# pk17r/online_3d_reconstruction

Measured on AMD Instinct MI355X. Metric: frames_per_sec, higher is better.
Workload: dtype f32; 1 GPU; synthetic 1280x720 dense stereo, jump_pixels 1, 200 frames/GPU, voxel_size 0.05, min_points_per_voxel 1, SOR off, frames resident in HBM (BASELINE.json configs[1]); frames_per_gpu=200, rows=720, cols=1280, jump_pixels=1, parallelism=frame-sharded x1

## Files before the change

### online_3d_reconstruction_amd/csrc/kernels/radix_sort.inc

```

__device__ __forceinline__ int64_t hist_at(bool tm, int dgt, int tile, int n_tiles)
{
    return tm ? (int64_t)tile * kMaxRadix + dgt : (int64_t)dgt * n_tiles + tile;
}

__global__ __launch_bounds__(kSortThreads) void k_radix_hist(const uint32_t* __restrict__ keys0,
                                                             const uint32_t* __restrict__ keys1, int64_t cap,
                                                             const VoxelGeom* __restrict__ geom, int pass,
                                                             int n_tiles, uint32_t* __restrict__ hist,
                                                             uint32_t* __restrict__ hist_part, int tm)
{
    constexpr int kSub = 4;
    __shared__ uint32_t h[kSub * kSortWaves * kMaxRadix];
    const int f = blockIdx.y, tile = blockIdx.x;
    const VoxelGeom g = geom[f];
    if (g.overflow || pass >= (int)g.passes) return;
    const uint32_t n = g.n;
    if ((int64_t)tile * kSortTile >= (int64_t)n) return;
    const int bins = geom_bins(g), shift = pass * (int)g.bpp;
    const uint32_t dmask = (uint32_t)bins - 1u;
    for (int i = threadIdx.x; i < kSub * kSortWaves * kMaxRadix; i += kSortThreads) h[i] = 0;
    __syncthreads();
    const uint32_t* src = (((pass + g.buf0) & 1) ? keys1 : keys0) + (int64_t)f * cap;
    const int64_t base = (int64_t)tile * kSortTile;
// ... 83 lines not shown
            dst[i] = key;
            atomicAdd(&hw[key & dmask], 1u);
        }
    }
    __syncthreads();
    uint32_t* hd = hist + (int64_t)f * kMaxRadix * n_tiles;
    for (int dgt = threadIdx.x; dgt < bins; dgt += kSortThreads) {
        uint32_t t = 0;
#pragma unroll
        for (int ww = 0; ww < kSub * kSortWaves; ++ww) t += h[ww * kMaxRadix + dgt];
        hd[hist_at(tm != 0, dgt, tile, n_tiles)] = t;
    }
}

constexpr int kCntStride = 17;
constexpr int kCntWords = kMaxRadix * kCntStride;
constexpr int kRankWords = kScatWaves * kCntWords;
struct ScatterLds {
    __attribute__((aligned(16))) uint32_t smem[kRankWords > 2 * kScatTile ? kRankWords : 2 * kScatTile];
    uint32_t wave_tot[kScatWaves * kMaxRadix];
    uint32_t local_base[kMaxRadix];
    uint32_t delta[kMaxRadix];
    uint32_t scan_lds[kScatWaves + 1];
};
struct ScatterJob {
    const uint32_t *kin, *vin;
    uint32_t *kout, *vout;
    const uint32_t* hist;
    const uint32_t* hist_part;
    int64_t begin, end;
    uint32_t dmask;
    int shift, bins, pass, n_tiles;
    bool tm;
};

__device__ __forceinline__ void emit_part_range(const uint32_t* __restrict__ tile_off, int n_emit_tiles, int tile, int part,
                                                int64_t n, int64_t& begin, int64_t& end)
{
    if (tile_off) {
        constexpr int kPer = kEmitGroup / kScatParts;
        const int e0 = (tile * kScatParts + part) * kPer;
        begin = tile_off[e0];
        end = e0 + kPer < n_emit_tiles ? (int64_t)tile_off[e0 + kPer] : n;
    } else {
        begin = (int64_t)tile * kSortTile + (int64_t)part * kScatTile;
        end = begin + kScatTile < n ? begin + kScatTile : n;
    }
}
typedef uint32_t u32x4_a4_t __attribute__((ext_vector_type(4), aligned(4)));

__device__ __forceinline__ void scatter_load(const ScatterJob& J, int tile, int part, uint32_t (&key)[kSortRounds],
                                             uint32_t (&val)[kSortRounds], uint32_t& gstart)
{
    const int lane = threadIdx.x & 63, w = threadIdx.x >> 6;
    const int64_t lbase = J.begin + (int64_t)w * kSortWaveItems + (int64_t)lane * kSortRounds;
    gstart = 0;
    if ((int)threadIdx.x < J.bins) {
        gstart = J.hist[hist_at(J.tm, threadIdx.x, tile, J.n_tiles)];
        if (part != 0) gstart += J.hist_part[hist_at(J.tm, threadIdx.x, tile, J.n_tiles)];
    }
    if (lbase + kSortRounds <= J.end) {
#pragma unroll
        for (int q = 0; q < kSortRounds / 4; ++q) {
            const u32x4_a4_t k4 = *reinterpret_cast<const u32x4_a4_t*>(J.kin + lbase + 4 * q);
            key[4 * q] = k4.x; key[4 * q + 1] = k4.y; key[4 * q + 2] = k4.z; key[4 * q + 3] = k4.w;
        }
        if (J.pass != 0) {
#pragma unroll
            for (int q = 0; q < kSortRounds / 4; ++q) {
                const u32x4_a4_t v4 = *reinterpret_cast<const u32x4_a4_t*>(J.vin + lbase + 4 * q);
                val[4 * q] = v4.x; val[4 * q + 1] = v4.y; val[4 * q + 2] = v4.z; val[4 * q + 3] = v4.w;
            }
        }
    } else {
#pragma unroll
        for (int r = 0; r < kSortRounds; ++r) {
            const int64_t i = lbase + r;
            const bool ok = i < J.end;
            key[r] = ok ? J.kin[i] : 0xffffffffu;
            val[r] = (J.pass != 0 && ok) ? J.vin[i] : 0u;
        }
    }
    if (J.pass == 0) {
#pragma unroll
        for (int r = 0; r < kSortRounds; ++r) val[r] = (uint32_t)(lbase + r);
    }
}

__device__ __forceinline__ void scatter_tile(const ScatterJob& J, ScatterLds& L, const uint32_t (&key)[kSortRounds],
                                             const uint32_t (&val)[kSortRounds], uint32_t gstart)
{
    uint32_t* smem = L.smem;
    uint32_t* stage = L.smem;
    const int lane = threadIdx.x & 63, w = threadIdx.x >> 6;
    const uint32_t cnt = (uint32_t)(J.end - J.begin);
    const int64_t lbase = J.begin + (int64_t)w * kSortWaveItems + (int64_t)lane * kSortRounds;
    const int shift = J.shift, bins = J.bins;
    const uint32_t dmask = J.dmask;
    for (int i = threadIdx.x; i < kRankWords; i += kScatThreads) smem[i] = 0;
    __syncthreads();

    uint32_t* cw = smem + w * kCntWords;
    const int quad = lane >> 2, sub = lane & 3;
    const uint32_t fsh = 7u * (uint32_t)sub;
    uint32_t own[kSortRounds];
#pragma unroll
    for (int r = 0; r < kSortRounds; ++r) {
        own[r] = 0;
        if (lbase + r < J.end) {
            const uint32_t dgt = (key[r] >> shift) & dmask;
            const uint32_t old = atomicAdd(&cw[dgt * kCntStride + quad], 1u << fsh);
            own[r] = (old >> fsh) & 127u;
        }
    }
    __builtin_amdgcn_wave_barrier();
#pragma unroll
    for (int h = 0; h < kMaxRadix / 64; ++h) {
        const int row = lane + 64 * h;
        if (row < bins) {
            uint32_t run = 0;
#pragma unroll
            for (int j = 0; j < 16; ++j) {
                const uint32_t v = cw[row * kCntStride + j];
                const uint32_t t = v + (v << 7);
                const uint32_t t2 = t + (t << 14);
                cw[row * kCntStride + j] = (run << 21) | (t2 & 0x1fffffu);
                run += (t2 >> 21) & 127u;
            }
            L.wave_tot[w * kMaxRadix + row] = run;
        }
    }
    __syncthreads();

    uint32_t tot = 0;
    const int dg = threadIdx.x;
    if (dg < bins) {
#pragma unroll
        for (int ww = 0; ww < kScatWaves; ++ww) {
            const uint32_t t = L.wave_tot[ww * kMaxRadix + dg];
            L.wave_tot[ww * kMaxRadix + dg] = tot;
            tot += t;
        }
    }
    uint32_t tile_total;
    const uint32_t lb = block_excl_scan_u32<kScatWaves>(tot, L.scan_lds, tile_total);
    if (dg < bins) {
        L.local_base[dg] = lb;
        L.delta[dg] = gstart - lb;
    }
    __syncthreads();

    uint32_t pos[kSortRounds];
    const uint32_t qsh = sub ? 7u * (uint32_t)(sub - 1) : 0u, qmk = sub ? 127u : 0u;
#pragma unroll
    for (int r = 0; r < kSortRounds; ++r) {
        if (lbase + r < J.end) {
            const uint32_t dgt = (key[r] >> shift) & dmask;
            const uint32_t v = cw[dgt * kCntStride + quad];
            pos[r] = L.local_base[dgt] + L.wave_tot[w * kMaxRadix + dgt] + (v >> 21) + ((v >> qsh) & qmk) + own[r];
        }
    }
    __syncthreads();
    uint32_t* stage_v = L.smem + kScatTile;
#pragma unroll
    for (int r = 0; r < kSortRounds; ++r) {
        if (lbase + r < J.end) {
            stage[pos[r]] = key[r];
            stage_v[pos[r]] = val[r];
        }
    }
    __syncthreads();
#pragma unroll
    for (int r = 0; r < kSortRounds; ++r) {
        const uint32_t p = r * kScatThreads + threadIdx.x;
        if (p < cnt) {
            const uint32_t k = stage[p];
            const uint32_t d = p + L.delta[(k >> shift) & dmask];
            J.kout[d] = k;
            J.vout[d] = stage_v[p];
        }
    }
}

__global__ __launch_bounds__(kScatThreads) void k_radix_scatter_lane(uint32_t* __restrict__ keys0, uint32_t* __restrict__ vals0,
                                                                     uint32_t* __restrict__ keys1, uint32_t* __restrict__ vals1,
                                                                     int64_t cap, const VoxelGeom* __restrict__ geom, int pass,
                                                                     int n_tiles, const uint32_t* __restrict__ hist_scanned,
                                                                     const uint32_t* __restrict__ hist_part, int tm,
                                                                     const uint32_t* __restrict__ emit_tile_off,
                                                                     int n_emit_tiles)
{
    __shared__ ScatterLds L;
    const int f = blockIdx.y;
    const VoxelGeom g = geom[f];
    if (g.overflow || pass >= (int)g.passes) return;
    const uint32_t* tile_off = emit_tile_off ? emit_tile_off + (int64_t)f * n_emit_tiles : nullptr;
    const int n_items = tile_off ? (n_emit_tiles + kEmitGroup / kScatParts - 1) / (kEmitGroup / kScatParts)
                                 : (int)(((int64_t)g.n + kScatTile - 1) / kScatTile);
    const int item = xcd_chunk_item(blockIdx.x, n_items);
    if (item < 0) return;
    const int tile = item / kScatParts, part = item % kScatParts;
    ScatterJob J;
    emit_part_range(tile_off, n_emit_tiles, tile, part, (int64_t)g.n, J.begin, J.end);
    if (J.begin >= J.end) return;
    const int par = (pass + (int)g.buf0) & 1;
    J.kin = (par ? keys1 : keys0) + (int64_t)f * cap;
    J.vin = (par ? vals1 : vals0) + (int64_t)f * cap;
    J.kout = (par ? keys0 : keys1) + (int64_t)f * cap;
    J.vout = (par ? vals0 : vals1) + (int64_t)f * cap;
    J.hist = hist_scanned + (int64_t)f * kMaxRadix * n_tiles;
    J.hist_part = hist_part + (int64_t)f * kMaxRadix * n_tiles;
    J.bins = geom_bins(g);
    J.dmask = (uint32_t)J.bins - 1u;
    J.shift = pass * (int)g.bpp;
    J.pass = pass;
    J.n_tiles = n_tiles;
    J.tm = tm != 0;
    uint32_t key0[kSortRounds], val0[kSortRounds], g0;
    scatter_load(J, tile, part, key0, val0, g0);
    scatter_tile(J, L, key0, val0, g0);
}
```

### online_3d_reconstruction_amd/csrc/kernels/voxel_runs.inc

```


constexpr int kHeadWaves = 4;
__global__ __launch_bounds__(kHeadWaves * kWave) void k_run_heads(const uint32_t* __restrict__ keys0, const uint32_t* __restrict__ keys1,
                                                                  int64_t cap, const VoxelGeom* __restrict__ geom, int n_tiles,
                                                                  uint32_t* __restrict__ seg_cnt, int buf_sel,
                                                                  uint8_t* __restrict__ head_bits)
{
    static_assert(kSegTile == 16 * kWave, "16 records per lane");
    const int f = blockIdx.y, lane = threadIdx.x & 63;
    const int tile = blockIdx.x * kHeadWaves + (threadIdx.x >> 6);
    const VoxelGeom g = geom[f];
    if (g.overflow || tile >= n_tiles) return;
    const int64_t n = g.n;
    const uint32_t* k = (buf_sel < 0 ? sorted_buf(g, keys0, keys1) : (buf_sel ? keys1 : keys0)) + (int64_t)f * cap;
    uint32_t c = 0;
    const int64_t i0 = (int64_t)tile * kSegTile + lane * 16;
    if ((int64_t)tile * kSegTile < n) {
        uint32_t kk[16];
        if (((((int64_t)f * cap) & 3) == 0) && i0 + 15 < n) {
#pragma unroll
            for (int q = 0; q < 4; ++q) {
                const uint4 v = *reinterpret_cast<const uint4*>(k + i0 + 4 * q);
                kk[4 * q] = v.x; kk[4 * q + 1] = v.y; kk[4 * q + 2] = v.z; kk[4 * q + 3] = v.w;
            }
        } else {
#pragma unroll
            for (int q = 0; q < 16; ++q) kk[q] = (i0 + q < n) ? k[i0 + q] : 0u;
        }
        uint32_t prev = (uint32_t)wave_shr1_i32((int32_t)kk[15]);
        if (lane == 0) prev = (i0 > 0 && i0 < n) ? k[i0 - 1] : 0u;
        uint32_t bits = 0;
#pragma unroll
        for (int q = 0; q < 16; ++q) {
            const int64_t i = i0 + q;
            if (i < n && (i == 0 || kk[q] != (q ? kk[q - 1] : prev))) bits |= 1u << ((q >> 2) * 8 + (q & 3));
        }
        reinterpret_cast<uint32_t*>(head_bits + ((int64_t)f * n_tiles + tile) * 256)[lane] = bits;
        c = (uint32_t)__popc(bits);
    }
    c = wave_sum_u32(c);
    if (lane == 0) seg_cnt[(int64_t)f * n_tiles + tile] = c;
}

constexpr int kStartWaves = 4;
__global__ __launch_bounds__(kStartWaves * kWave) void k_run_starts(
    const uint32_t* __restrict__ keys0, const uint32_t* __restrict__ keys1, int64_t cap, const VoxelGeom* __restrict__ geom,
    int n_tiles, const uint32_t* __restrict__ seg_off, const uint32_t* __restrict__ n_vox, uint32_t* __restrict__ seg_start,
    int buf_sel, uint32_t* __restrict__ head_keys_out, const VoxelGeom* __restrict__ mode, const o3dr_point* __restrict__ in_pts,
    float z_offset, const uint8_t* __restrict__ head_bits)
{
    static_assert(kSegTile == 16 * kWave, "16 records per lane");
    const int f = blockIdx.y, lane = threadIdx.x & 63;
    const int tile = blockIdx.x * kStartWaves + (threadIdx.x >> 6);
    const VoxelGeom g = geom[f];
    if (g.overflow) return;
    if (mode && mode[f].grouped == 0u) return;
    const uint32_t n = g.n;
    const int64_t base = (int64_t)tile * kSegTile;
// ... 64 lines not shown
    const int f = blockIdx.y, tile = blockIdx.x;
    if (geom[f].overflow || geom[f].grouped != 0u) return;
    const uint32_t nv = n_vox[f];
    const int64_t base = (int64_t)tile * kSegTile;
    if (base >= nv) return;
    const uint32_t* ss = seg_start + (int64_t)f * (cap + 1);
    uint32_t* ki = keep_idx + (int64_t)f * cap;
    uint32_t off = seg_off[(int64_t)f * n_tiles + tile];
    for (int j = 0; j < kSegTile / 256; ++j) {
        const int64_t o = base + j * 256 + threadIdx.x;
        const bool keep = (o < nv) && (ss[o + 1] - ss[o] >= min_points);
        uint32_t total;
        const uint32_t pos = block_excl_scan_u32<4>(keep ? 1u : 0u, scan_lds, total);
        if (keep) ki[off + pos] = (uint32_t)o;
        off += total;
    }
}

__global__ __launch_bounds__(256) void k_frame_offsets(const VoxelGeom* __restrict__ geom, const uint32_t* __restrict__ n_vox,
                                                       const uint32_t* __restrict__ n_keep,
                                                       const uint32_t* __restrict__ n_grp, int frames, int passthrough,
                                                       uint32_t* __restrict__ n_out, uint64_t* __restrict__ out_off,
                                                       CloudCounters* __restrict__ cc, SortStats* __restrict__ stats,
                                                       const VoxelGeom* __restrict__ sort_geom)
{
    __shared__ uint32_t scan_lds[5];
    __shared__ unsigned long long acc[6];
    if (threadIdx.x < 6) acc[threadIdx.x] = 0;
    __syncthreads();
    const uint64_t base = cc->count;
    uint64_t carry = 0;
    for (int f0 = 0; f0 < frames; f0 += 256) {
        const int f = f0 + threadIdx.x;
        uint32_t m = 0;
        if (f < frames) {
            const VoxelGeom g = geom[f];
            if (passthrough) {
                m = g.n;
            } else if (g.overflow) {
                m = g.n;
                atomicOr(&acc[3], (unsigned long long)O3DR_STATUS_VOXEL_OVERFLOW);
            } else {
                m = (n_grp && sort_geom[f].grouped) ? n_grp[f] : (n_keep ? n_keep[f] : n_vox[f]);
                atomicAdd(&acc[0], (unsigned long long)sort_geom[f].n * g.passes);
                atomicAdd(&acc[5], (unsigned long long)sort_geom[f].n);
                atomicAdd(&acc[1], (unsigned long long)g.n);
                atomicAdd(&acc[2], (unsigned long long)m);
            }
        }
        uint32_t total;
        const uint32_t excl = block_excl_scan_u32<4>(m, scan_lds, total);
        if (f < frames) {
            n_out[f] = m;
            out_off[f] = base + carry + excl;
        }
        carry += total;
    }
    __syncthreads();
    if (threadIdx.x == 0) {
        cc->count = base + carry;
        cc->status |= (uint32_t)acc[3];
        if (stats) {
            stats->sort_record_passes += acc[0];
            stats->voxel_points_in += acc[1];
            stats->voxel_points_out += acc[2];
            stats->sort_records += acc[5];
        }
    }
}

__global__ void k_test_corrupt_payload(uint32_t* __restrict__ vals0, uint32_t* __restrict__ vals1, const VoxelGeom* __restrict__ geom)
{
    const VoxelGeom g = geom[0];
    if (g.overflow || g.n == 0u) return;
    uint32_t* v = ((g.passes + g.buf0) & 1u) ? vals1 : vals0;
    v[g.n / 2u] = 0xfffffff0u;
}

__device__ __forceinline__ void centroid_block(int64_t bx, int f, const VoxelGeom& g, uint32_t n_o,
                                               const o3dr_point* __restrict__ in, int64_t in_fstride,
                                               const uint32_t* __restrict__ vals0, const uint32_t* __restrict__ vals1,
                                               int64_t cap, const uint32_t* __restrict__ seg_start,
                                               const uint32_t* __restrict__ keep_idx, const uint64_t* __restrict__ out_off,
                                               float z_offset, int passthrough, o3dr_point* __restrict__ out_base,
                                               float* __restrict__ out_mm, int nbx, CloudCounters* __restrict__ cc,
                                               const CloudHeads& ch)
{
    const int64_t o = bx * kPtThreads + threadIdx.x;
    const bool active = o < (int64_t)n_o;
// ... 418 lines not shown
```

### online_3d_reconstruction_amd/csrc/o3dr_api.hip

```cpp
#include <dlfcn.h>
#include <stdio.h>
#include <stdlib.h>
#include <string.h>

#include <algorithm>
#include <cfloat>
#include <chrono>
#include <cmath>
#include <condition_variable>
#include <mutex>
#include <string>
#include <vector>

#include <rccl/rccl.h>

#include "../../include/o3dr_testing.h"
#include "o3dr_device.h"
#include "o3dr_image_stack.h"
#include "o3dr_profile.h"

using namespace o3dr;

static thread_local std::string g_err;
static int fail(int code, const char* what)
// ... 193 lines not shown
        sort_tiles > c->ws_sort_tiles || seg_tiles > c->ws_seg_tiles || mm_floats > c->ws_mm_floats) {
        const size_t MM = mm_floats > c->ws_mm_floats ? mm_floats : c->ws_mm_floats;
        const size_t E = elems > c->ws_elems ? elems : c->ws_elems;
        const int F = frames > c->ws_frames ? frames : c->ws_frames;
        const size_t TE = emit_tiles > c->ws_emit_tiles ? emit_tiles : c->ws_emit_tiles;
        const size_t TS = sort_tiles > c->ws_sort_tiles ? sort_tiles : c->ws_sort_tiles;
        const size_t TG = seg_tiles > c->ws_seg_tiles ? seg_tiles : c->ws_seg_tiles;
        Workspace& w = c->ws;
        const size_t boxes = E / 64 + 8 * (size_t)F + 64;
        CHK(carve(c, c->ws_block, [&](Carve& k) {
            k.take(w.keys[0], E);
            k.take(w.keys[1], E);
            k.take(w.vals[0], E);
            k.take(w.vals[1], E);
            k.take(w.seg_start, E);
            k.take(w.keep_idx, E);
            k.take(w.run_start, E);
            k.take(w.grp_cnt, (E > (size_t)kGroupMinSlots ? E : (size_t)kGroupMinSlots) / kGroupCells + 2);
            k.take(w.tile_cnt, TE);
            k.take(w.hist, TS * kMaxRadix);
            k.take(w.hist_part, TS * kMaxRadix);
            k.take(w.seg_cnt, TG);
            k.take(w.head_bits, TG * 256);
            k.take(w.scan_partial, (TS * kMaxRadix + TG + TE + E) / 4096 + 8 * (size_t)F + 16);
            k.take(w.mm, MM);
            k.take(w.n_valid, (size_t)F);
            k.take(w.n_kp, (size_t)F);
            k.take(w.n_vox, (size_t)F);
            k.take(w.n_out, (size_t)F);
            k.take(w.out_off, (size_t)F);
            k.take(w.geom, (size_t)F);
            k.take(w.geom_runs, (size_t)F);
            k.take(w.n_runs, (size_t)F);
            k.take(w.n_grp_out, (size_t)F);
            k.take(w.out_mm, boxes * 6);
            k.take(w.out_mm_partial, (size_t)kBoxFoldBlocks * 6);
            k.take(w.wave_gc, boxes * 6);
            w.bytes = k.off;
        }));
        c->ws_elems = E;
        c->ws_frames = F;
        c->ws_emit_tiles = TE;
        c->ws_sort_tiles = TS;
        c->ws_seg_tiles = TG;
        c->ws_mm_floats = MM;
    }
// ... 1279 lines not shown
            launch_reproject(&c->prof, c->stream, a, nb, c->ws.pts, c->ws.tile_cnt, c->ws.n_kp, c->ws.n_valid, c->ws.mm,
                             c->ws.scan_partial);
        VoxelArgs v;
        v.keys_ready = fused ? 1 : 0;
        v.emit_tiles = emit_tiles;
        v.cloud_box = c->cloud_box_valid ? c->cloud_box : nullptr;
        heads_for_append(c, v);
        v.in = c->ws.pts;
        v.in_fstride = cap;
        v.n_dev = c->ws.n_valid;
        v.frames = nb;
        v.cap = cap;
        v.leaf[0] = leaf[0];
        v.leaf[1] = leaf[1];
        v.leaf[2] = leaf[2];
        v.min_points = mp;
        v.z_offset = zo;
        v.out_base = c->cloud_big;
        v.cc = c->cc_big;
        v.passthrough = c->params.dont_downsample ? 1 : 0;
        v.mm_used = a.n_tiles + 1;
        v.stats = c->stats_dev;
        v.use_runs = 0;
        if (with_sor) {
            v.mm_used = launch_sor(&c->prof, c->stream, c->ws, c->ws.pts, cap, c->ws.n_valid, nb, cap, a.n_tiles + 1, 1.0, c->ws.sor_pts,
                                   cap, c->ws.sor_n);
            v.in = c->ws.sor_pts;
            v.n_dev = c->ws.sor_n;
        }
        launch_voxel_grid(&c->prof, c->stream, c->ws, v);
        HIPCHK(hipGetLastError());
        c->cloud_ub += (int64_t)nb * cap;
        c->cloud_n_exact = false;
        if (streaming) HIPCHK(hipEventRecord(c->ev_done[slot], c->stream));
    }
    if (streaming) HIPCHK(hipStreamSynchronize(c->stream));
    return O3DR_OK;
}

extern "C" int o3dr_accumulate_frames(o3dr_ctx* c, const uint8_t* disp, int64_t disp_frame_stride, int64_t disp_pitch,
                                      const uint8_t* bgr, int64_t bgr_frame_stride, int64_t bgr_pitch, int32_t rows,
                                      int32_t cols, const float* poses, int32_t n_frames, int32_t mem)
{
    return accumulate_impl(c, disp, disp_frame_stride, disp_pitch, bgr, bgr_frame_stride, bgr_pitch, rows, cols, poses, n_frames,
                           nullptr, nullptr, mem);
}
// ... 3902 lines not shown
    if (total_ms) *total_ms = c->prof.total_ms[kernel_id];
    if (launches) *launches = c->prof.launches[kernel_id];
    return O3DR_OK;
}
extern "C" int o3dr_profile_reset(o3dr_ctx* c)
{
    CTX_ENTER(c);
    HIPCHK(hipMemsetAsync(c->stats_dev, 0, sizeof(SortStats), c->stream));
    HIPCHK(hipStreamSynchronize(c->stream));
    c->prof.reset();
    return O3DR_OK;
}
extern "C" int o3dr_profile_stats(o3dr_ctx* c, int64_t out[8])
{
    CTX_ENTER(c);
    if (!out) return fail(O3DR_ERR_INVALID_ARG, "out is NULL");
    HIPCHK(hipMemcpyAsync(c->stats_host, c->stats_dev, sizeof(SortStats), hipMemcpyDeviceToHost, c->stream));
    HIPCHK(hipStreamSynchronize(c->stream));
    out[0] = (int64_t)c->stats_host->sort_record_passes;
    out[1] = (int64_t)c->stats_host->voxel_points_in;
    out[2] = (int64_t)c->stats_host->voxel_points_out;
    out[3] = 0;
    out[4] = (int64_t)c->stats_host->sort_records;
    out[5] = out[6] = out[7] = 0;
    return O3DR_OK;
}
extern "C" int o3dr_device_info(o3dr_ctx* c, char* name, int32_t name_len, int32_t* cu_count, int64_t* hbm_bytes)
{
    CTX_ENTER(c);
    hipDeviceProp_t p;
    HIPCHK(hipGetDeviceProperties(&p, c->device));
    if (name && name_len > 0) snprintf(name, (size_t)name_len, "%s (%s)", p.name, p.gcnArchName);
    if (cu_count) *cu_count = p.multiProcessorCount;
    if (hbm_bytes) *hbm_bytes = (int64_t)p.totalGlobalMem;
    return O3DR_OK;
}
```

### online_3d_reconstruction_amd/csrc/o3dr_device.h

```cpp
#pragma once
#include <hip/hip_runtime.h>
#include <stdint.h>

#include "../../include/o3dr.h"

namespace o3dr {

constexpr int kWave = 64;
constexpr int kEmitThreads = 256;
constexpr int kEmitPerLane = 4;
constexpr int kEmitTile = kEmitThreads * kEmitPerLane;
constexpr int kSortWaves = 8;
constexpr int kSortThreads = kSortWaves * kWave;
constexpr int kSortRounds = 16;
constexpr int kSortWaveItems = kSortRounds * kWave;
constexpr int kSortTile = kSortWaves * kSortWaveItems;
constexpr int kScatParts = 2;
constexpr int kScatWaves = kSortWaves / kScatParts;
constexpr int kScatThreads = kScatWaves * kWave;
constexpr int kScatTile = kScatWaves * kSortWaveItems;
constexpr int kEmitGroup = kSortTile / kEmitTile;
static_assert(kEmitGroup * kEmitTile == kSortTile && kEmitGroup % kScatParts == 0, "a scatter part is a whole number of emit tiles");
constexpr int kMaxRadixBits = 7;
constexpr int kMaxRadix = 1 << kMaxRadixBits;
constexpr int kMaxPasses = 5;
static_assert(kMaxRadix <= 2 * kSortThreads, "k_radix_scatter handles two digits per thread");
constexpr int kSlabClasses = 4;
constexpr int kXcds = 8;
constexpr int kPtThreads = 256;
constexpr int kSegTile = 1024;
constexpr int kMinmaxBlocks = 1024;
constexpr int kPartWords = 8;
constexpr int kSmallMax = 8192;
constexpr int kGroupBits = 5;
constexpr int kGroupCells = 1 << kGroupBits;
static_assert(kGroupCells <= kWave, "one lane per voxel of a group");
constexpr int kGroupWaves = 4;
constexpr int kGroupMinRunNum = 5, kGroupMinRunDen = 4;
constexpr int64_t kGroupMinCloud = 1 << 20;
constexpr int64_t kGroupMinSlots = 1 << 20;

struct VoxelGeom {
    float inv[3];
    int32_t min_b[3];
    int32_t div_b[3];
    uint32_t mul1, mul2;
    uint32_t overflow;
    uint32_t n;
    uint32_t passes;
// ... 34 lines not shown
    double min_disp;
    int32_t min_disp_u8;
    int64_t out_fstride;
    int64_t mm_stride;
    const QLutEntry* lut;
    int32_t disp_f64;
    float slab_inv[3];
    int32_t slab_shift;
};

struct Workspace {
    int32_t frames = 0;
    int64_t cap = 0;
    int32_t n_emit_tiles = 0, n_sort_tiles = 0, n_seg_tiles = 0;
    o3dr_point* pts = nullptr;
    uint32_t* keys[2] = {nullptr, nullptr};
    uint32_t* vals[2] = {nullptr, nullptr};
    uint32_t* seg_start = nullptr;
    uint32_t* tile_cnt = nullptr;
    uint32_t* hist = nullptr;
    uint32_t* hist_part = nullptr;
    uint32_t* seg_cnt = nullptr;
    uint8_t* head_bits = nullptr;
    uint32_t* scan_partial = nullptr;
    SorGeom* sor_geom = nullptr;
    float4* sor_xyz = nullptr;
    float* sor_dist = nullptr;
    uint32_t* sor_cell_first = nullptr;
    float2* sor_cell_z = nullptr;
    uint32_t sor_max_cells = 0;
    double* sor_partial = nullptr;
    o3dr_point* sor_pts = nullptr;
    uint32_t* sor_n = nullptr;
    uint32_t* sor_left = nullptr;
    uint32_t* sor_left_cnt = nullptr;
    int64_t sor_cap = 0;
    uint32_t* keep_idx = nullptr;
    uint32_t* run_start = nullptr;
    uint32_t* grp_cnt = nullptr;
    int64_t grp_slots = 0;
    uint32_t* n_runs = nullptr;
    uint32_t* n_grp_out = nullptr;
    VoxelGeom* geom_runs = nullptr;
    float* out_mm = nullptr;
    float* out_mm_partial = nullptr;
    int32_t* wave_gc = nullptr;
    float* mm = nullptr;
    int64_t mm_stride = 0;
    uint32_t* n_valid = nullptr;
    uint32_t* n_kp = nullptr;
    uint32_t* n_vox = nullptr;
    uint32_t* n_out = nullptr;
    uint64_t* out_off = nullptr;
    VoxelGeom* geom = nullptr;
    size_t bytes = 0;
};

struct SortStats {
    uint64_t sort_record_passes;
    uint64_t voxel_points_in;
    uint64_t voxel_points_out;
    uint64_t reserved;
    uint64_t sort_records;
    uint64_t pad[3];
};

struct CloudHeads {
    uint32_t* flags;
    float inv[3];
    float z_offset;
    int32_t* wave_gc;
};

struct CloudCounters {
    uint64_t count;
    uint32_t status;
    uint32_t pad;
};

struct IncGroup {
    int32_t bx, iy, iz;
    uint32_t mask;
};
struct IncCell {
    float s[7];
    uint32_t n;
};
// ... 461 lines not shown
```

### online_3d_reconstruction_amd/csrc/o3dr_kernels.hip

```cpp
#include <string.h>

#include "o3dr_device.h"
#include "o3dr_profile.h"

namespace o3dr {

#include "kernels/util.inc"
#include "kernels/reproject.inc"
#include "kernels/bookkeeping.inc"
#include "kernels/prepass.inc"
#include "kernels/voxel_index.inc"
#include "kernels/radix_sort.inc"
#include "kernels/voxel_runs.inc"
#include "kernels/incremental.inc"
#include "kernels/multigpu.inc"
#include "kernels/sor.inc"
#include "kernels/small.inc"
#include "kernels/nn.inc"
#include "kernels/mls.inc"
#include "kernels/cell_order.inc"
#include "kernels/plane.inc"
#include "kernels/mesh.inc"
#include "kernels/raster.inc"
#include "kernels/match.inc"
// ... 231 lines not shown
            }
            {
                ProfScope ps(pf, O3DR_K_OTHER, s);
                launch_scan(s, ws.seg_cnt, n_seg_tiles, n_seg_tiles, F, ws.n_runs, nullptr, ws.scan_partial);
            }
            {
                ProfScope ps(pf, O3DR_K_SEGMENT, s);
                k_run_geom<<<cdiv64(F, 64), 64, 0, s>>>(ws.geom, ws.n_runs, F, ws.geom_runs, v.use_runs > 1 ? 1 : 0, grp_slots);
                k_run_starts<<<dim3(cdiv64(n_seg_tiles, kStartWaves), F), kStartWaves * kWave, 0, s>>>(
                    ws.keys[0], ws.keys[1], cap, ws.geom, n_seg_tiles, ws.seg_cnt, ws.n_runs, ws.run_start, 0, ws.keys[1],
                    ws.geom_runs, v.in, v.z_offset, hb);
            }
            {
                ProfScope ps(pf, O3DR_K_KEYGEN, s);
                k_voxel_keys_hist0<<<grid, kSortThreads, 0, s>>>(v.in, v.in_fstride, ws.geom, v.z_offset, cap, ws.keys[0],
                                                                 n_sort_tiles, ws.hist, ws.hist_part, ws.geom_runs, tm);
            }
        } else if (!v.keys_ready) {
            ProfScope ps(pf, O3DR_K_KEYGEN, s);
            k_voxel_keys_hist0<<<grid, kSortThreads, 0, s>>>(v.in, v.in_fstride, ws.geom, v.z_offset, cap, ws.keys[0],
                                                             n_sort_tiles, ws.hist, ws.hist_part, nullptr, tm);
        }
        const int64_t hist_row = (int64_t)kMaxRadix * n_sort_tiles;

        for (int pass = 0; pass < kMaxPasses; ++pass) {
            const bool emit_tiles = pass == 0 && v.emit_tiles > 0;
            if (!(pass == 0 && ((!use_runs && !v.keys_ready) || emit_tiles))) {
                ProfScope ps(pf, O3DR_K_SORT_HIST, s);
                k_radix_hist<<<grid, kSortThreads, 0, s>>>(ws.keys[0], ws.keys[1], cap, sort_geom, pass, n_sort_tiles,
                                                          ws.hist, ws.hist_part, tm);
            }
            {
                ProfScope ps(pf, O3DR_K_OTHER, s);
                if (tm)
                    k_scan_hist_tm<<<F, 1024, tm_lds, s>>>(ws.hist, sort_geom, pass, n_sort_tiles, emit_tiles ? 1 : 0);
                else
                    launch_scan(s, ws.hist, hist_row, hist_row, F, nullptr, nullptr, ws.scan_partial, sort_geom, pass,
                                n_sort_tiles);
            }
            {
                ProfScope ps(pf, O3DR_K_SORT_SCATTER, s);
                k_radix_scatter_lane<<<dim3(xcd_grid((int64_t)n_sort_tiles * kScatParts), F), kScatThreads, 0, s>>>(
                    ws.keys[0], ws.vals[0], ws.keys[1], ws.vals[1], cap, sort_geom, pass, n_sort_tiles, ws.hist, ws.hist_part, tm,
                    emit_tiles ? ws.tile_cnt : nullptr, v.emit_tiles);
            }
        }
        const dim3 sgrid(n_seg_tiles, F);
        {
            ProfScope ps(pf, O3DR_K_SEGMENT, s);
            k_run_heads<<<dim3(cdiv64(n_seg_tiles, kHeadWaves), F), kHeadWaves * kWave, 0, s>>>(ws.keys[0], ws.keys[1], cap, sort_geom, n_seg_tiles,
                                                                                       ws.seg_cnt, -1, ws.head_bits);
        }
        {
            ProfScope ps(pf, O3DR_K_OTHER, s);
            launch_scan(s, ws.seg_cnt, n_seg_tiles, n_seg_tiles, F, ws.n_vox, nullptr, ws.scan_partial);
        }
        {
            ProfScope ps(pf, O3DR_K_SEGMENT, s);
            k_run_starts<<<dim3(cdiv64(n_seg_tiles, kStartWaves), F), kStartWaves * kWave, 0, s>>>(ws.keys[0], ws.keys[1], cap, sort_geom, n_seg_tiles, ws.seg_cnt, ws.n_vox,
                                              ws.seg_start, -1, nullptr, nullptr, nullptr, 0.f, ws.head_bits);
        }
        if (v.min_points > 1) {
            {
                ProfScope ps(pf, O3DR_K_SEGMENT, s);
                k_keep_count<<<sgrid, 256, 0, s>>>(ws.seg_start, cap, sort_geom, ws.n_vox, v.min_points, n_seg_tiles, ws.seg_cnt);
            }
            {
                ProfScope ps(pf, O3DR_K_OTHER, s);
                launch_scan(s, ws.seg_cnt, n_seg_tiles, n_seg_tiles, F, ws.n_out, nullptr, ws.scan_partial);
            }
            {
                ProfScope ps(pf, O3DR_K_SEGMENT, s);
                k_keep_write<<<sgrid, 256, 0, s>>>(ws.seg_start, cap, sort_geom, ws.n_vox, v.min_points, n_seg_tiles, ws.seg_cnt,
                                                  ws.keep_idx);
// ... 5 lines not shown
        k_test_corrupt_payload<<<1, 1, 0, s>>>(ws.vals[0], ws.vals[1], sort_geom);
    if (cap > 0 && use_runs) {
        {
            ProfScope ps(pf, O3DR_K_OTHER, s);
            (void)hipMemsetAsync(ws.grp_cnt, 0, sizeof(uint32_t) * (size_t)(max_groups + 1), s);
        }
        {
            ProfScope ps(pf, O3DR_K_CENTROID_RUNS, s);
            int64_t nwg = cdiv64(max_groups < cap ? max_groups : cap, kGroupWaves);
            if (nwg > 16384) nwg = 16384;
            if (nwg < 1) nwg = 1;
            k_centroid_groups<<<(int)nwg, kGroupWaves * kWave, 0, s>>>(
                v.in, ws.keys[0], ws.keys[1], ws.vals[0], ws.vals[1], ws.seg_start, ws.run_start, ws.geom_runs, ws.geom, ws.n_vox,
                v.z_offset, v.min_points, reinterpret_cast<uint4*>(ws.pts), grp_slots, ws.grp_cnt, v.cc);
        }
        {
            ProfScope ps(pf, O3DR_K_OTHER, s);
            launch_scan(s, ws.grp_cnt, max_groups + 1, max_groups + 1, 1, ws.n_grp_out, nullptr, ws.scan_partial);
        }
    }
    {
        ProfScope ps(pf, O3DR_K_OTHER, s);
        k_frame_offsets<<<1, 256, 0, s>>>(ws.geom, ws.n_vox, n_keep, use_runs ? ws.n_grp_out : nullptr, F, v.passthrough,
                                          ws.n_out, ws.out_off, v.cc, v.stats, sort_geom);
    }
    const int nbx = cdiv64(cap, kPtThreads);
    if (cap > 0 && use_runs) {
        ProfScope ps(pf, O3DR_K_CENTROID_RUNS, s);
        int64_t nwg = cdiv64(cap, 256);
        if (nwg > 8192) nwg = 8192;
        k_group_compact<<<(int)nwg, 256, 0, s>>>(v.in, ws.geom_runs, ws.geom, ws.n_vox, ws.grp_cnt,
                                                reinterpret_cast<const uint4*>(ws.pts), ws.out_off, v.z_offset, v.out_base);
    }
    if (cap > 0) {
        ProfScope ps(pf, O3DR_K_CENTROID, s);
        float* out_mm = v.cloud_box ? ws.out_mm : nullptr;
        CloudHeads heads = v.cloud_heads;
        heads.wave_gc = ws.wave_gc;
        const uint32_t* keep = (v.min_points > 1 && !v.passthrough) ? ws.keep_idx : nullptr;
        if (use_runs)
            k_centroid<true><<<dim3(nbx < 4096 ? nbx : 4096, F), kPtThreads, 0, s>>>(
                v.in, v.in_fstride, ws.vals[0], ws.vals[1], cap, ws.seg_start, keep, ws.geom_runs, ws.n_out, ws.out_off,
                v.z_offset, v.passthrough, v.out_base, out_mm, nbx, v.cc, CloudHeads{nullptr, {0.f, 0.f, 0.f}, 0.f, nullptr});
        else
            k_centroid<false><<<dim3(xcd_grid(nbx), F), kPtThreads, 0, s>>>(
                v.in, v.in_fstride, ws.vals[0], ws.vals[1], cap, ws.seg_start, keep, ws.geom, ws.n_out, ws.out_off,
                v.z_offset, v.passthrough, v.out_base, out_mm, nbx, v.cc, heads);
// ... 41 lines not shown
        ProfScope ps(pf, O3DR_K_SEGMENT, s);
        k_run_geom<<<1, 64, 0, s>>>(ws.geom, ws.n_runs, 1, ws.geom_runs, 1, INT64_MAX);
        k_run_starts<<<dim3(cdiv64(n_seg_tiles, kStartWaves), 1), kStartWaves * kWave, 0, s>>>(
            ws.keys[0], ws.keys[1], cap, ws.geom, n_seg_tiles, ws.seg_cnt, ws.n_runs, ws.run_start, 0, ws.keys[1], ws.geom_runs, in,
            z_offset, ws.head_bits);
    }
    const dim3 grid(n_sort_tiles, 1);
    const int64_t hist_row = (int64_t)kMaxRadix * n_sort_tiles;
    for (int pass = 0; pass < kMaxPasses; ++pass) {
        {
            ProfScope ps(pf, O3DR_K_SORT_HIST, s);
            k_radix_hist<<<grid, kSortThreads, 0, s>>>(ws.keys[0], ws.keys[1], cap, sort_geom, pass, n_sort_tiles, ws.hist, ws.hist_part, tm);
        }
        {
            ProfScope ps(pf, O3DR_K_OTHER, s);
            if (tm)
                k_scan_hist_tm<<<1, 1024, tm_lds, s>>>(ws.hist, sort_geom, pass, n_sort_tiles, 0);
            else
                launch_scan(s, ws.hist, hist_row, hist_row, 1, nullptr, nullptr, ws.scan_partial, sort_geom, pass, n_sort_tiles);
        }
        {
            ProfScope ps(pf, O3DR_K_SORT_SCATTER, s);
            k_radix_scatter_lane<<<dim3(xcd_grid((int64_t)n_sort_tiles * kScatParts), 1), kScatThreads, 0, s>>>(
                ws.keys[0], ws.vals[0], ws.keys[1], ws.vals[1], cap, sort_geom, pass, n_sort_tiles, ws.hist, ws.hist_part, tm, nullptr, 0);
        }
    }
    {
        ProfScope ps(pf, O3DR_K_SEGMENT, s);
        k_run_heads<<<dim3(cdiv64(n_seg_tiles, kHeadWaves), 1), kHeadWaves * kWave, 0, s>>>(ws.keys[0], ws.keys[1], cap, sort_geom,
                                                                                             n_seg_tiles, ws.seg_cnt, -1, ws.head_bits);
    }
    {
        ProfScope ps(pf, O3DR_K_OTHER, s);
        launch_scan(s, ws.seg_cnt, n_seg_tiles, n_seg_tiles, 1, ws.n_vox, nullptr, ws.scan_partial);
    }
    {
        ProfScope ps(pf, O3DR_K_SEGMENT, s);
        k_run_starts<<<dim3(cdiv64(n_seg_tiles, kStartWaves), 1), kStartWaves * kWave, 0, s>>>(
            ws.keys[0], ws.keys[1], cap, sort_geom, n_seg_tiles, ws.seg_cnt, ws.n_vox, ws.seg_start, -1, nullptr, nullptr, nullptr, 0.f,
            ws.head_bits);
    }
    if (test_corrupt) k_test_corrupt_payload<<<1, 1, 0, s>>>(ws.vals[0], ws.vals[1], sort_geom);
}

void launch_inc_fold(Profiler* pf, hipStream_t s, Workspace& ws, const o3dr_point* in, float z_offset, const IncFoldArgs& a,
                     uint32_t* partial)
{
    {
        ProfScope ps(pf, O3DR_K_CENTROID_RUNS, s);
        int64_t nwg = cdiv64(a.nt, kGroupWaves);
        if (nwg > 16384) nwg = 16384;
        if (nwg < 1) nwg = 1;
        k_inc_fold<<<(int)nwg, kGroupWaves * kWave, 0, s>>>(in, ws.keys[0], ws.keys[1], ws.vals[0], ws.vals[1], ws.seg_start, ws.run_start,
// ... 343 lines not shown
}
void launch_partition(Profiler* pf, hipStream_t s, Workspace& ws, const VoxelArgs& v, int n_parts, o3dr_point* out,
                      uint64_t* counts_dev, uint32_t* overflow_dev, const void* hdrs_dev, int n_hdrs)
{
    launch_partition_count(pf, s, ws, v, n_parts, counts_dev, overflow_dev, hdrs_dev, n_hdrs);
    launch_partition_move(pf, s, ws, v, n_parts, out, nullptr);
}

static void launch_radix_passes(Workspace& ws, hipStream_t s, int64_t cap, int passes, int frames = 1)
{
    const int F = frames;
    const int n_sort_tiles = cdiv64(cap, kSortTile);
    const int64_t hist_row = (int64_t)kMaxRadix * n_sort_tiles;
    const size_t tm_lds = hist_tm_lds(n_sort_tiles);
    const int tm = hist_tm(n_sort_tiles);
    for (int pass = 0; pass < passes && pass < kMaxPasses; ++pass) {
        k_radix_hist<<<dim3(n_sort_tiles, F), kSortThreads, 0, s>>>(ws.keys[0], ws.keys[1], cap, ws.geom, pass, n_sort_tiles, ws.hist,
                                                                    ws.hist_part, tm);
        if (tm)
            k_scan_hist_tm<<<F, 1024, tm_lds, s>>>(ws.hist, ws.geom, pass, n_sort_tiles, 0);
        else
            launch_scan(s, ws.hist, hist_row, hist_row, F, nullptr, nullptr, ws.scan_partial, ws.geom, pass, n_sort_tiles);
        k_radix_scatter_lane<<<dim3(xcd_grid((int64_t)n_sort_tiles * kScatParts), F), kScatThreads, 0, s>>>(
            ws.keys[0], ws.vals[0], ws.keys[1], ws.vals[1], cap, ws.geom, pass, n_sort_tiles, ws.hist, ws.hist_part, tm, nullptr, 0);
    }
}

void launch_search_grid(Workspace& ws, hipStream_t s, const o3dr_point* in, int64_t in_fstride, const uint32_t* n_dev, int frames,
                        int64_t cap, int mm_used, double cell_points, uint32_t active_above)
{
    const int F = frames;
    const int64_t cell_stride = (int64_t)ws.sor_max_cells + 1;
    uint32_t max_cells = (uint32_t)(cap / 2 > 1024 ? cap / 2 : 1024);
    if (max_cells > ws.sor_max_cells) max_cells = ws.sor_max_cells;
    int cell_bits = 1;
    while ((1u << cell_bits) < max_cells) ++cell_bits;
    const int sort_passes = (cell_bits + kMaxRadixBits - 1) / kMaxRadixBits;
    k_sor_plan<<<F, 256, 0, s>>>(ws.mm, ws.mm_stride, mm_used, n_dev, max_cells, ws.sor_geom, ws.geom, cell_points, active_above);
    (void)hipMemsetAsync(ws.sor_cell_first, 0, (size_t)F * (size_t)cell_stride * 4, s);
    k_sor_cells<<<dim3(cdiv64(cap, 256), F), 256, 0, s>>>(in, in_fstride, ws.sor_geom, cap, ws.keys[0]);
    launch_radix_passes(ws, s, cap, sort_passes, F);
    k_sor_cell_counts<<<dim3(cdiv64(cap, 256), F), 256, 0, s>>>(ws.keys[0], ws.keys[1], ws.geom, ws.sor_geom, cap, cell_stride, ws.sor_cell_first);
    launch_scan(s, ws.sor_cell_first, cell_stride, cell_stride, F, nullptr, nullptr, ws.scan_partial);
    k_sor_gather<<<dim3(cdiv64(cap, 256), F), 256, 0, s>>>(in, in_fstride, ws.vals[0], ws.vals[1], ws.sor_geom, ws.geom, cap, ws.sor_xyz);
}

int launch_sor(Profiler* pf, hipStream_t s, Workspace& ws, const o3dr_point* in, int64_t in_fstride, const uint32_t* n_dev,
// ... 297 lines not shown
```

Baseline: 34890 frames/s.

## Emit segment head flags from the last radix scatter pass instead of sorted keys

On the final radix pass, the scatter kernel now writes a one-byte head flag per record into a side buffer instead of writing the sorted keys. Heads are found by comparing neighbours in the LDS stage, plus an LDS bitmask of which digits the previous tile's tail shares. A new k_side_heads kernel packs these bytes into head_bits and seg_cnt, and k_run_heads skips frames that went through this path. This removes the final key write and the separate key re-read for head detection. In exchange it adds atomics, a possible backward-scan loop in one wave, and extra byte traffic, and correctness depends on the cross-tile boundary logic.

```diff
diff --git a/online_3d_reconstruction_amd/csrc/kernels/radix_sort.inc b/online_3d_reconstruction_amd/csrc/kernels/radix_sort.inc
--- a/online_3d_reconstruction_amd/csrc/kernels/radix_sort.inc
+++ b/online_3d_reconstruction_amd/csrc/kernels/radix_sort.inc
@@ -129,10 +129,14 @@
     uint32_t local_base[kMaxRadix];
     uint32_t delta[kMaxRadix];
     uint32_t scan_lds[kScatWaves + 1];
+    uint32_t hmask[8];
+    uint32_t lmin;
 };
 struct ScatterJob {
     const uint32_t *kin, *vin;
     uint32_t *kout, *vout;
+    uint8_t* heads;
+    uint32_t low_mask;
     const uint32_t* hist;
     const uint32_t* hist_part;
     int64_t begin, end;
@@ -157,11 +161,16 @@
 typedef uint32_t u32x4_a4_t __attribute__((ext_vector_type(4), aligned(4)));
 
 __device__ __forceinline__ void scatter_load(const ScatterJob& J, int tile, int part, uint32_t (&key)[kSortRounds],
-                                             uint32_t (&val)[kSortRounds], uint32_t& gstart)
+                                             uint32_t (&val)[kSortRounds], uint32_t& gstart, uint32_t& back)
 {
     const int lane = threadIdx.x & 63, w = threadIdx.x >> 6;
     const int64_t lbase = J.begin + (int64_t)w * kSortWaveItems + (int64_t)lane * kSortRounds;
     gstart = 0;
+    back = 0;
+    if (J.heads && w == kScatWaves - 1) {
+        const int64_t j = J.begin - kWave + lane;
+        if (j >= 0) back = J.kin[j];
+    }
     if ((int)threadIdx.x < J.bins) {
         gstart = J.hist[hist_at(J.tm, threadIdx.x, tile, J.n_tiles)];
         if (part != 0) gstart += J.hist_part[hist_at(J.tm, threadIdx.x, tile, J.n_tiles)];
@@ -195,7 +204,7 @@
 }
 
 __device__ __forceinline__ void scatter_tile(const ScatterJob& J, ScatterLds& L, const uint32_t (&key)[kSortRounds],
-                                             const uint32_t (&val)[kSortRounds], uint32_t gstart)
+                                             const uint32_t (&val)[kSortRounds], uint32_t gstart, uint32_t back)
 {
     uint32_t* smem = L.smem;
     uint32_t* stage = L.smem;
@@ -205,7 +214,13 @@
     const int shift = J.shift, bins = J.bins;
     const uint32_t dmask = J.dmask;
     for (int i = threadIdx.x; i < kRankWords; i += kScatThreads) smem[i] = 0;
-    __syncthreads();
+    if (J.heads) {
+        if (threadIdx.x < 8) L.hmask[threadIdx.x] = 0;
+        if (threadIdx.x == 0) L.lmin = key[0] & J.low_mask;
+    }
+    __syncthreads();
+    const volatile uint32_t* hmask = L.hmask;
+    const uint32_t lmin = J.heads ? L.lmin : 0u;
 
     uint32_t* cw = smem + w * kCntWords;
     const int quad = lane >> 2, sub = lane & 3;
@@ -218,6 +233,8 @@
             const uint32_t dgt = (key[r] >> shift) & dmask;
             const uint32_t old = atomicAdd(&cw[dgt * kCntStride + quad], 1u << fsh);
             own[r] = (old >> fsh) & 127u;
+            if (J.heads && (key[r] & J.low_mask) == lmin && !((hmask[4 + (dgt >> 5)] >> (dgt & 31u)) & 1u))
+                atomicOr(&L.hmask[4 + (dgt >> 5)], 1u << (dgt & 31u));
         }
     }
     __builtin_amdgcn_wave_barrier();
@@ -238,6 +255,25 @@
         }
     }
     __syncthreads();
+    if (J.heads && w == kScatWaves - 1) {
+        int64_t j0 = J.begin - kWave;
+        uint32_t kb = back;
+        for (;;) {
+            const bool in = j0 + lane >= 0 && (kb & J.low_mask) == lmin;
+            if (in) {
+                const uint32_t dgt = (kb >> shift) & dmask;
+                atomicOr(&L.hmask[dgt >> 5], 1u << (dgt & 31u));
+            }
+            __builtin_amdgcn_wave_barrier();
+            if (__ballot(in) != ~0ull || j0 <= 0) break;
+            uint32_t miss = 0;
+#pragma unroll
+            for (int q = 0; q < 4; ++q) miss |= hmask[4 + q] & ~hmask[q];
+            if (miss == 0u) break;
+            j0 -= kWave;
+            kb = j0 + lane >= 0 ? J.kin[j0 + lane] : 0u;
+        }
+    }
 
     uint32_t tot = 0;
     const int dg = threadIdx.x;
@@ -282,9 +318,19 @@
         const uint32_t p = r * kScatThreads + threadIdx.x;
         if (p < cnt) {
             const uint32_t k = stage[p];
-            const uint32_t d = p + L.delta[(k >> shift) & dmask];
-            J.kout[d] = k;
+            const uint32_t dgt = (k >> shift) & dmask;
+            const uint32_t d = p + L.delta[dgt];
             J.vout[d] = stage_v[p];
+            if (J.heads) {
+                bool head;
+                if (p != L.local_base[dgt])
+                    head = k != stage[p - 1];
+                else
+                    head = !((k & J.low_mask) == lmin && ((hmask[dgt >> 5] >> (dgt & 31u)) & 1u));
+                J.heads[d] = head ? 1 : 0;
+            } else {
+                J.kout[d] = k;
+            }
         }
     }
 }
@@ -295,7 +341,8 @@
                                                                      int n_tiles, const uint32_t* __restrict__ hist_scanned,
                                                                      const uint32_t* __restrict__ hist_part, int tm,
                                                                      const uint32_t* __restrict__ emit_tile_off,
-                                                                     int n_emit_tiles)
+                                                                     int n_emit_tiles, uint8_t* __restrict__ side,
+                                                                     int64_t side_stride)
 {
     __shared__ ScatterLds L;
     const int f = blockIdx.y;
@@ -323,7 +370,9 @@
     J.pass = pass;
     J.n_tiles = n_tiles;
     J.tm = tm != 0;
-    uint32_t key0[kSortRounds], val0[kSortRounds], g0;
-    scatter_load(J, tile, part, key0, val0, g0);
-    scatter_tile(J, L, key0, val0, g0);
-}
+    J.heads = (side && pass + 1 == (int)g.passes) ? side + (int64_t)f * side_stride : nullptr;
+    J.low_mask = (1u << J.shift) - 1u;
+    uint32_t key0[kSortRounds], val0[kSortRounds], g0, back;
+    scatter_load(J, tile, part, key0, val0, g0, back);
+    scatter_tile(J, L, key0, val0, g0, back);
+}
diff --git a/online_3d_reconstruction_amd/csrc/kernels/voxel_runs.inc b/online_3d_reconstruction_amd/csrc/kernels/voxel_runs.inc
--- a/online_3d_reconstruction_amd/csrc/kernels/voxel_runs.inc
+++ b/online_3d_reconstruction_amd/csrc/kernels/voxel_runs.inc
@@ -4,13 +4,14 @@
 __global__ __launch_bounds__(kHeadWaves * kWave) void k_run_heads(const uint32_t* __restrict__ keys0, const uint32_t* __restrict__ keys1,
                                                                   int64_t cap, const VoxelGeom* __restrict__ geom, int n_tiles,
                                                                   uint32_t* __restrict__ seg_cnt, int buf_sel,
-                                                                  uint8_t* __restrict__ head_bits)
+                                                                  uint8_t* __restrict__ head_bits, int side_heads)
 {
     static_assert(kSegTile == 16 * kWave, "16 records per lane");
     const int f = blockIdx.y, lane = threadIdx.x & 63;
     const int tile = blockIdx.x * kHeadWaves + (threadIdx.x >> 6);
     const VoxelGeom g = geom[f];
     if (g.overflow || tile >= n_tiles) return;
+    if (side_heads && g.passes != 0u) return;
     const int64_t n = g.n;
     const uint32_t* k = (buf_sel < 0 ? sorted_buf(g, keys0, keys1) : (buf_sel ? keys1 : keys0)) + (int64_t)f * cap;
     uint32_t c = 0;
@@ -34,6 +35,42 @@
         for (int q = 0; q < 16; ++q) {
             const int64_t i = i0 + q;
             if (i < n && (i == 0 || kk[q] != (q ? kk[q - 1] : prev))) bits |= 1u << ((q >> 2) * 8 + (q & 3));
+        }
+        reinterpret_cast<uint32_t*>(head_bits + ((int64_t)f * n_tiles + tile) * 256)[lane] = bits;
+        c = (uint32_t)__popc(bits);
+    }
+    c = wave_sum_u32(c);
+    if (lane == 0) seg_cnt[(int64_t)f * n_tiles + tile] = c;
+}
+
+__global__ __launch_bounds__(kHeadWaves * kWave) void k_side_heads(const uint8_t* __restrict__ side, int64_t side_stride,
+                                                                   const VoxelGeom* __restrict__ geom, int n_tiles,
+                                                                   uint32_t* __restrict__ seg_cnt, uint8_t* __restrict__ head_bits)
+{
+    static_assert(kSegTile == 16 * kWave, "16 records per lane");
+    const int f = blockIdx.y, lane = threadIdx.x & 63;
+    const int tile = blockIdx.x * kHeadWaves + (threadIdx.x >> 6);
+    const VoxelGeom g = geom[f];
+    if (g.overflow || g.passes == 0u || tile >= n_tiles) return;
+    const int64_t n = g.n;
+    const uint8_t* sb = side + (int64_t)f * side_stride;
+    uint32_t c = 0;
+    const int64_t i0 = (int64_t)tile * kSegTile + lane * 16;
+    if ((int64_t)tile * kSegTile < n) {
+        uint32_t w4[4] = {0u, 0u, 0u, 0u};
+        if (i0 + 15 < n) {
+            const uint4 v = stream_load_u4(reinterpret_cast<const uint4*>(sb + i0));
+            w4[0] = v.x; w4[1] = v.y; w4[2] = v.z; w4[3] = v.w;
+        } else {
+#pragma unroll
+            for (int q = 0; q < 16; ++q)
+                if (i0 + q < n) w4[q >> 2] |= (uint32_t)(sb[i0 + q] & 1u) << ((q & 3) * 8);
+        }
+        uint32_t bits = 0;
+#pragma unroll
+        for (int q = 0; q < 4; ++q) {
+            const uint32_t w = w4[q];
+            bits |= ((w & 1u) | ((w >> 7) & 2u) | ((w >> 14) & 4u) | ((w >> 21) & 8u)) << (8 * q);
         }
         reinterpret_cast<uint32_t*>(head_bits + ((int64_t)f * n_tiles + tile) * 256)[lane] = bits;
         c = (uint32_t)__popc(bits);
@@ -144,7 +181,7 @@
                                                        const uint32_t* __restrict__ n_grp, int frames, int passthrough,
                                                        uint32_t* __restrict__ n_out, uint64_t* __restrict__ out_off,
                                                        CloudCounters* __restrict__ cc, SortStats* __restrict__ stats,
-                                                       const VoxelGeom* __restrict__ sort_geom)
+                                                       const VoxelGeom* __restrict__ sort_geom, int side_heads)
 {
     __shared__ uint32_t scan_lds[5];
     __shared__ unsigned long long acc[6];
@@ -166,6 +203,7 @@
                 m = (n_grp && sort_geom[f].grouped) ? n_grp[f] : (n_keep ? n_keep[f] : n_vox[f]);
                 atomicAdd(&acc[0], (unsigned long long)sort_geom[f].n * g.passes);
                 atomicAdd(&acc[5], (unsigned long long)sort_geom[f].n);
+                if (side_heads && g.passes != 0u) atomicAdd(&acc[4], (unsigned long long)sort_geom[f].n);
                 atomicAdd(&acc[1], (unsigned long long)g.n);
                 atomicAdd(&acc[2], (unsigned long long)m);
             }
@@ -187,6 +225,7 @@
             stats->voxel_points_in += acc[1];
             stats->voxel_points_out += acc[2];
             stats->sort_records += acc[5];
+            stats->side_head_records += acc[4];
         }
     }
 }
diff --git a/online_3d_reconstruction_amd/csrc/o3dr_api.hip b/online_3d_reconstruction_amd/csrc/o3dr_api.hip
--- a/online_3d_reconstruction_amd/csrc/o3dr_api.hip
+++ b/online_3d_reconstruction_amd/csrc/o3dr_api.hip
@@ -239,6 +239,7 @@
             k.take(w.hist_part, TS * kMaxRadix);
             k.take(w.seg_cnt, TG);
             k.take(w.head_bits, TG * 256);
+            k.take(w.side, E + 16 * (size_t)F);
             k.take(w.scan_partial, (TS * kMaxRadix + TG + TE + E) / 4096 + 8 * (size_t)F + 16);
             k.take(w.mm, MM);
             k.take(w.n_valid, (size_t)F);
@@ -1564,6 +1565,8 @@
         v.mm_used = a.n_tiles + 1;
         v.stats = c->stats_dev;
         v.use_runs = 0;
+        v.test_corrupt = c->test_corrupt;
+        c->test_corrupt = 0;
         if (with_sor) {
             v.mm_used = launch_sor(&c->prof, c->stream, c->ws, c->ws.pts, cap, c->ws.n_valid, nb, cap, a.n_tiles + 1, 1.0, c->ws.sor_pts,
                                    cap, c->ws.sor_n);
@@ -5512,7 +5515,8 @@
     out[2] = (int64_t)c->stats_host->voxel_points_out;
     out[3] = 0;
     out[4] = (int64_t)c->stats_host->sort_records;
-    out[5] = out[6] = out[7] = 0;
+    out[5] = (int64_t)c->stats_host->side_head_records;
+    out[6] = out[7] = 0;
     return O3DR_OK;
 }
 extern "C" int o3dr_device_info(o3dr_ctx* c, char* name, int32_t name_len, int32_t* cu_count, int64_t* hbm_bytes)
diff --git a/online_3d_reconstruction_amd/csrc/o3dr_device.h b/online_3d_reconstruction_amd/csrc/o3dr_device.h
--- a/online_3d_reconstruction_amd/csrc/o3dr_device.h
+++ b/online_3d_reconstruction_amd/csrc/o3dr_device.h
@@ -25,6 +25,7 @@
 constexpr int kMaxRadix = 1 << kMaxRadixBits;
 constexpr int kMaxPasses = 5;
 static_assert(kMaxRadix <= 2 * kSortThreads, "k_radix_scatter handles two digits per thread");
+static inline int64_t side_frame_stride(int64_t cap) { return (cap + 15) & ~(int64_t)15; }
 constexpr int kSlabClasses = 4;
 constexpr int kXcds = 8;
 constexpr int kPtThreads = 256;
@@ -105,6 +106,7 @@
     uint32_t* hist_part = nullptr;
     uint32_t* seg_cnt = nullptr;
     uint8_t* head_bits = nullptr;
+    uint8_t* side = nullptr;
     uint32_t* scan_partial = nullptr;
     SorGeom* sor_geom = nullptr;
     float4* sor_xyz = nullptr;
@@ -145,7 +147,8 @@
     uint64_t voxel_points_out;
     uint64_t reserved;
     uint64_t sort_records;
-    uint64_t pad[3];
+    uint64_t side_head_records;
+    uint64_t pad[2];
 };
 
 struct CloudHeads {
diff --git a/online_3d_reconstruction_amd/csrc/o3dr_kernels.hip b/online_3d_reconstruction_amd/csrc/o3dr_kernels.hip
--- a/online_3d_reconstruction_amd/csrc/o3dr_kernels.hip
+++ b/online_3d_reconstruction_amd/csrc/o3dr_kernels.hip
@@ -277,7 +277,8 @@
                                                              n_sort_tiles, ws.hist, ws.hist_part, nullptr, tm);
         }
         const int64_t hist_row = (int64_t)kMaxRadix * n_sort_tiles;
-
+        uint8_t* const side = use_runs ? nullptr : ws.side;
+        const int64_t side_stride = side_frame_stride(cap);
         for (int pass = 0; pass < kMaxPasses; ++pass) {
             const bool emit_tiles = pass == 0 && v.emit_tiles > 0;
             if (!(pass == 0 && ((!use_runs && !v.keys_ready) || emit_tiles))) {
@@ -297,14 +298,17 @@
                 ProfScope ps(pf, O3DR_K_SORT_SCATTER, s);
                 k_radix_scatter_lane<<<dim3(xcd_grid((int64_t)n_sort_tiles * kScatParts), F), kScatThreads, 0, s>>>(
                     ws.keys[0], ws.vals[0], ws.keys[1], ws.vals[1], cap, sort_geom, pass, n_sort_tiles, ws.hist, ws.hist_part, tm,
-                    emit_tiles ? ws.tile_cnt : nullptr, v.emit_tiles);
+                    emit_tiles ? ws.tile_cnt : nullptr, v.emit_tiles, side, side_stride);
             }
         }
         const dim3 sgrid(n_seg_tiles, F);
         {
             ProfScope ps(pf, O3DR_K_SEGMENT, s);
             k_run_heads<<<dim3(cdiv64(n_seg_tiles, kHeadWaves), F), kHeadWaves * kWave, 0, s>>>(ws.keys[0], ws.keys[1], cap, sort_geom, n_seg_tiles,
-                                                                                       ws.seg_cnt, -1, ws.head_bits);
+                                                                                       ws.seg_cnt, -1, ws.head_bits, side != nullptr);
+            if (side)
+                k_side_heads<<<dim3(cdiv64(n_seg_tiles, kHeadWaves), F), kHeadWaves * kWave, 0, s>>>(side, side_stride, sort_geom, n_seg_tiles,
+                                                                                            ws.seg_cnt, ws.head_bits);
         }
         {
             ProfScope ps(pf, O3DR_K_OTHER, s);
@@ -356,7 +360,8 @@
     {
         ProfScope ps(pf, O3DR_K_OTHER, s);
         k_frame_offsets<<<1, 256, 0, s>>>(ws.geom, ws.n_vox, n_keep, use_runs ? ws.n_grp_out : nullptr, F, v.passthrough,
-                                          ws.n_out, ws.out_off, v.cc, v.stats, sort_geom);
+                                          ws.n_out, ws.out_off, v.cc, v.stats, sort_geom,
+                                          (!use_runs && ws.side && !v.passthrough && cap > 0) ? 1 : 0);
     }
     const int nbx = cdiv64(cap, kPtThreads);
     if (cap > 0 && use_runs) {
@@ -444,13 +449,14 @@
         {
             ProfScope ps(pf, O3DR_K_SORT_SCATTER, s);
             k_radix_scatter_lane<<<dim3(xcd_grid((int64_t)n_sort_tiles * kScatParts), 1), kScatThreads, 0, s>>>(
-                ws.keys[0], ws.vals[0], ws.keys[1], ws.vals[1], cap, sort_geom, pass, n_sort_tiles, ws.hist, ws.hist_part, tm, nullptr, 0);
+                ws.keys[0], ws.vals[0], ws.keys[1], ws.vals[1], cap, sort_geom, pass, n_sort_tiles, ws.hist, ws.hist_part, tm, nullptr, 0,
+                nullptr, 0);
         }
     }
     {
         ProfScope ps(pf, O3DR_K_SEGMENT, s);
         k_run_heads<<<dim3(cdiv64(n_seg_tiles, kHeadWaves), 1), kHeadWaves * kWave, 0, s>>>(ws.keys[0], ws.keys[1], cap, sort_geom,
-                                                                                             n_seg_tiles, ws.seg_cnt, -1, ws.head_bits);
+                                                                                             n_seg_tiles, ws.seg_cnt, -1, ws.head_bits, 0);
     }
     {
         ProfScope ps(pf, O3DR_K_OTHER, s);
@@ -840,7 +846,8 @@
         else
             launch_scan(s, ws.hist, hist_row, hist_row, F, nullptr, nullptr, ws.scan_partial, ws.geom, pass, n_sort_tiles);
         k_radix_scatter_lane<<<dim3(xcd_grid((int64_t)n_sort_tiles * kScatParts), F), kScatThreads, 0, s>>>(
-            ws.keys[0], ws.vals[0], ws.keys[1], ws.vals[1], cap, ws.geom, pass, n_sort_tiles, ws.hist, ws.hist_part, tm, nullptr, 0);
+            ws.keys[0], ws.vals[0], ws.keys[1], ws.vals[1], cap, ws.geom, pass, n_sort_tiles, ws.hist, ws.hist_part, tm, nullptr, 0,
+            nullptr, 0);
     }
 }
 
```

Measured after the change: 35430 frames/s (median of 6 runs). +1.5%, better.
